# Medical-Image-Analysis-Laboratory/MSLesions3D

Measured on AMD Instinct MI355X. Metric: training volumes/sec at 128^3 batch-4 (fwd+loss+bwd+Adam), data-parallel over N MI355X, higher is better.
Workload: dtype f32; 1 GPU; 128^3 synthetic volumes, batch 4/GPU, 1 channel(s), fp32, SSD3D+MobileNet3D full train step (BASELINE configs[1]); global_batch=4, parallelism=dp1, priors=9344

## Files before the change

mslesions3d_amd/csrc/pwconv.hip:

```cpp
#include "common.hpp"
#include <algorithm>
#include <cstdlib>

namespace {

typedef float f32x16 __attribute__((ext_vector_type(16)));

constexpr int BM = 64, BN = 128, BK = 32;
constexpr int FOLD_MAXK = 512;
constexpr int WS_LD = BK + 1;

template <bool AFFINE, bool STATS, bool TRANS_W>
__global__ __launch_bounds__(256) void pw_gemm_kernel(const float* __restrict__ X,
                                                      const float* __restrict__ in_scale,
                                                      const float* __restrict__ in_shift,
                                                      const float* __restrict__ Wt, float* __restrict__ Y,
                                                      double* __restrict__ partials, int M, int K, int S,
                                                      msl::BnFold fold) {
  __shared__ __align__(16) float Xs[BK][BN];
  __shared__ float Ws[BM][WS_LD];
  __shared__ float red[2][2][BM];
  __shared__ float f_sc[AFFINE ? FOLD_MAXK : 1], f_sh[AFFINE ? FOLD_MAXK : 1];
  const int n = blockIdx.z, m0 = blockIdx.y * BM, s0 = blockIdx.x * BN;
  const int tid = threadIdx.x, lane = tid & 63, wv = tid >> 6;
  const int wm = wv >> 1, wn = wv & 1;
  const float* Xn = X + (size_t)n * K * S;
  const bool vec_ok = (S & 3) == 0;

  float4 xr[4], wr[2];
  auto load_chunk = [&](int k0) {
    if (vec_ok) {
#pragma unroll
      for (int i = 0; i < 4; ++i)
        xr[i] = msl::load4_zfill<true>(Xn + (size_t)(k0 + (tid >> 5) + i * 8) * S, s0 + (tid & 31) * 4, S);
    } else {
#pragma unroll
      for (int i = 0; i < 4; ++i)
        xr[i] = msl::load4_zfill<false>(Xn + (size_t)(k0 + (tid >> 5) + i * 8) * S, s0 + (tid & 31) * 4, S);
    }
#pragma unroll
    for (int i = 0; i < 2; ++i) {
      if (!TRANS_W) {
        const int m = (tid >> 3) + i * 32, k4 = (tid & 7) * 4;
        wr[i] = *reinterpret_cast<const float4*>(Wt + (size_t)(m0 + m < M ? m0 + m : 0) * K + k0 + k4);
      } else {
        const int k = (tid >> 4) + i * 16, m4 = (tid & 15) * 4;
        wr[i] = *reinterpret_cast<const float4*>(Wt + (size_t)(k0 + k) * M + (m0 + m4 < M ? m0 + m4 : 0));
      }
    }
  };
  auto store_chunk = [&](int k0) {
#pragma unroll
    for (int i = 0; i < 4; ++i) {
      const int r = (tid >> 5) + i * 8, c4 = (tid & 31) * 4, col = s0 + c4;
      float4 v = xr[i];
      if (AFFINE) {
        const float sc = f_sc[k0 + r], sh = f_sh[k0 + r];
        v.x = col < S ? msl::act(v.x, sc, sh) : 0.f;
        v.y = col + 1 < S ? msl::act(v.y, sc, sh) : 0.f;
        v.z = col + 2 < S ? msl::act(v.z, sc, sh) : 0.f;
        v.w = col + 3 < S ? msl::act(v.w, sc, sh) : 0.f;
      }
      *reinterpret_cast<float4*>(&Xs[r][c4]) = v;
    }
#pragma unroll
    for (int i = 0; i < 2; ++i) {
      const float4 v = wr[i];
      if (!TRANS_W) {
        const int m = (tid >> 3) + i * 32, k4 = (tid & 7) * 4;
        Ws[m][k4] = v.x; Ws[m][k4 + 1] = v.y; Ws[m][k4 + 2] = v.z; Ws[m][k4 + 3] = v.w;
      } else {
        const int k = (tid >> 4) + i * 16, m4 = (tid & 15) * 4;
        Ws[m4][k] = v.x; Ws[m4 + 1][k] = v.y; Ws[m4 + 2][k] = v.z; Ws[m4 + 3][k] = v.w;
      }
    }
  };

  f32x16 acc0 = {0}, acc1 = {0};
  load_chunk(0);
  if (AFFINE) {
    if (fold.partials) {
      msl::bn_fold_block(fold, 0, K, f_sc, f_sh);
    } else {
      for (int k = threadIdx.x; k < K && k < FOLD_MAXK; k += blockDim.x) {
        f_sc[k] = in_scale[k];
        f_sh[k] = in_shift[k];
      }
    }
  }
  for (int k0 = 0; k0 < K; k0 += BK) {
    __syncthreads();
    store_chunk(k0);
    __syncthreads();
    if (k0 + BK < K) load_chunk(k0 + BK);
#pragma unroll
    for (int kk = 0; kk < BK / 2; ++kk) {
      const int kr = 2 * kk + (lane >> 5);
      const float a = Ws[wm * 32 + (lane & 31)][kr];
      const float b0 = Xs[kr][wn * 64 + (lane & 31)];
      const float b1 = Xs[kr][wn * 64 + 32 + (lane & 31)];
      acc0 = __builtin_amdgcn_mfma_f32_32x32x2f32(a, b0, acc0, 0, 0, 0);
      acc1 = __builtin_amdgcn_mfma_f32_32x32x2f32(a, b1, acc1, 0, 0, 0);
    }
  }

  float* Yn = Y + (size_t)n * M * S;
  const int colbase = s0 + wn * 64 + (lane & 31);
#pragma unroll
  for (int r = 0; r < 16; ++r) {
    const int row = m0 + wm * 32 + (r & 3) + 8 * (r >> 2) + 4 * (lane >> 5);
    if (row < M && colbase < S) Yn[(size_t)row * S + colbase] = acc0[r];
    if (row < M && colbase + 32 < S) Yn[(size_t)row * S + colbase + 32] = acc1[r];
  }
  if (STATS) {
#pragma unroll
    for (int r = 0; r < 16; ++r) {
      float s = acc0[r] + acc1[r];
      float q = fmaf(acc0[r], acc0[r], acc1[r] * acc1[r]);
#pragma unroll
      for (int m = 16; m > 0; m >>= 1) {
        s += __shfl_xor(s, m, 64);
        q += __shfl_xor(q, m, 64);
      }
      if ((lane & 31) == 0) {
        const int row = wm * 32 + (r & 3) + 8 * (r >> 2) + 4 * (lane >> 5);
        red[0][wn][row] = s;
        red[1][wn][row] = q;
      }
    }
    __syncthreads();
    if (tid < BM && m0 + tid < M && partials) {
      const int NP = gridDim.z * gridDim.x, p = n * gridDim.x + blockIdx.x;
      partials[(size_t)(m0 + tid) * NP + p] = (double)red[0][0][tid] + (double)red[0][1][tid];
      partials[((size_t)M + m0 + tid) * NP + p] = (double)red[1][0][tid] + (double)red[1][1][tid];
    }
  }
}

constexpr int KS_BM = 32, KS_BN = 64;
constexpr int KS_WAVE_LDS = BK * KS_BN + KS_BM * WS_LD;

template <bool AFFINE, bool STATS, bool TRANS_W, int NW>
__global__ __launch_bounds__(NW * 64) void pw_gemm_ksplit_kernel(const float* __restrict__ X,
                                                             const float* __restrict__ in_scale,
                                                             const float* __restrict__ in_shift,
                                                             const float* __restrict__ Wt, float* __restrict__ Y,
                                                             double* __restrict__ partials, int M, int K, int S,
                                                             msl::BnFold fold) {
  extern __shared__ __align__(16) float lds[];
  __shared__ float f_sc[AFFINE ? FOLD_MAXK : 1], f_sh[AFFINE ? FOLD_MAXK : 1];
  const int n = blockIdx.z, m0 = blockIdx.y * KS_BM, s0 = blockIdx.x * KS_BN;
  const int tid = threadIdx.x, lane = tid & 63, wv = tid >> 6;
  float* Xs = lds + wv * KS_WAVE_LDS;
  float* Ws = Xs + BK * KS_BN;
  const float* Xn = X + (size_t)n * K * S;
  const bool vec_ok = (S & 3) == 0;
  const int kq = K / NW;
  const int kbeg = wv * kq;
  const int nchunks = kq / BK;

  float4 xr[8], wr[4];
  auto load_chunk = [&](int k0) {
    if (vec_ok) {
#pragma unroll
      for (int i = 0; i < 8; ++i)
        xr[i] = msl::load4_zfill<true>(Xn + (size_t)(k0 + (lane >> 4) + i * 4) * S, s0 + (lane & 15) * 4, S);
    } else {
#pragma unroll
      for (int i = 0; i < 8; ++i)
        xr[i] = msl::load4_zfill<false>(Xn + (size_t)(k0 + (lane >> 4) + i * 4) * S, s0 + (lane & 15) * 4, S);
    }
#pragma unroll
    for (int i = 0; i < 4; ++i) {
      if (!TRANS_W) {
        const int m = (lane >> 3) + i * 8, k4 = (lane & 7) * 4;
        wr[i] = *reinterpret_cast<const float4*>(Wt + (size_t)(m0 + m < M ? m0 + m : 0) * K + k0 + k4);
      } else {
        const int k = (lane >> 3) + i * 8, m4 = (lane & 7) * 4;
        wr[i] = *reinterpret_cast<const float4*>(Wt + (size_t)(k0 + k) * M + (m0 + m4 < M ? m0 + m4 : 0));
      }
    }
  };
  auto store_chunk = [&](int k0) {
#pragma unroll
    for (int i = 0; i < 8; ++i) {
      const int r = (lane >> 4) + i * 4, c4 = (lane & 15) * 4, col = s0 + c4;
      float4 v = xr[i];
      if (AFFINE) {
        const float sc = f_sc[k0 + r], sh = f_sh[k0 + r];
        v.x = col < S ? msl::act(v.x, sc, sh) : 0.f;
        v.y = col + 1 < S ? msl::act(v.y, sc, sh) : 0.f;
        v.z = col + 2 < S ? msl::act(v.z, sc, sh) : 0.f;
        v.w = col + 3 < S ? msl::act(v.w, sc, sh) : 0.f;
      }
      *reinterpret_cast<float4*>(Xs + r * KS_BN + c4) = v;
    }
#pragma unroll
    for (int i = 0; i < 4; ++i) {
      if (!TRANS_W) {
        const int m = (lane >> 3) + i * 8, k4 = (lane & 7) * 4;
        float* d = Ws + m * WS_LD + k4;
        d[0] = wr[i].x; d[1] = wr[i].y; d[2] = wr[i].z; d[3] = wr[i].w;
      } else {
        const int k = (lane >> 3) + i * 8, m4 = (lane & 7) * 4;
        Ws[(m4 + 0) * WS_LD + k] = wr[i].x; Ws[(m4 + 1) * WS_LD + k] = wr[i].y;
        Ws[(m4 + 2) * WS_LD + k] = wr[i].z; Ws[(m4 + 3) * WS_LD + k] = wr[i].w;
      }
    }
  };

  f32x16 acc0 = {0}, acc1 = {0};
  load_chunk(kbeg);
  if (AFFINE) {
    if (fold.partials) {
      msl::bn_fold_block(fold, 0, K, f_sc, f_sh);
    } else {
      for (int k = threadIdx.x; k < K && k < FOLD_MAXK; k += blockDim.x) {
        f_sc[k] = in_scale[k];
        f_sh[k] = in_shift[k];
      }
    }
  }
  for (int ch = 0; ch < nchunks; ++ch) {
    __syncthreads();
    store_chunk(kbeg + ch * BK);
    __syncthreads();
    if (ch + 1 < nchunks) load_chunk(kbeg + (ch + 1) * BK);
#pragma unroll
    for (int kk = 0; kk < BK / 2; ++kk) {
      const int kr = 2 * kk + (lane >> 5);
      const float a = Ws[(lane & 31) * WS_LD + kr];
      const float b0 = Xs[kr * KS_BN + (lane & 31)];
      const float b1 = Xs[kr * KS_BN + 32 + (lane & 31)];
      acc0 = __builtin_amdgcn_mfma_f32_32x32x2f32(a, b0, acc0, 0, 0, 0);
      acc1 = __builtin_amdgcn_mfma_f32_32x32x2f32(a, b1, acc1, 0, 0, 0);
    }
  }
  __syncthreads();
  constexpr int RLD = KS_BN + 1;
  for (int half = NW / 2; half >= 1; half >>= 1) {
    if (wv >= half && wv < 2 * half) {
      float* slot = lds + (wv - half) * (KS_BM * RLD);
#pragma unroll
      for (int r = 0; r < 16; ++r) {
        const int row = (r & 3) + 8 * (r >> 2) + 4 * (lane >> 5);
        slot[row * RLD + (lane & 31)] = acc0[r];
        slot[row * RLD + 32 + (lane & 31)] = acc1[r];
      }
    }
    __syncthreads();
    if (wv < half) {
      const float* slot = lds + wv * (KS_BM * RLD);
#pragma unroll
      for (int r = 0; r < 16; ++r) {
        const int row = (r & 3) + 8 * (r >> 2) + 4 * (lane >> 5);
        acc0[r] += slot[row * RLD + (lane & 31)];
        acc1[r] += slot[row * RLD + 32 + (lane & 31)];
      }
    }
    __syncthreads();
  }
  if (wv != 0) return;
  float* Yn = Y + (size_t)n * M * S;
  const int colbase = s0 + (lane & 31);
#pragma unroll
  for (int r = 0; r < 16; ++r) {
    const int rl = (r & 3) + 8 * (r >> 2) + 4 * (lane >> 5);
    const int row = m0 + rl;
    const float v0 = acc0[r];
    const float v1 = acc1[r];
    if (row < M && colbase < S) Yn[(size_t)row * S + colbase] = v0;
    if (row < M && colbase + 32 < S) Yn[(size_t)row * S + colbase + 32] = v1;
    if (STATS) {
      float s = v0 + v1;
      float q = fmaf(v0, v0, v1 * v1);
#pragma unroll
      for (int m = 16; m > 0; m >>= 1) {
        s += __shfl_xor(s, m, 64);
        q += __shfl_xor(q, m, 64);
      }
      if ((lane & 31) == 0 && row < M && partials) {
        const int NP = gridDim.z * gridDim.x, p = n * gridDim.x + blockIdx.x;
        partials[(size_t)row * NP + p] = (double)s;
        partials[((size_t)M + row) * NP + p] = (double)q;
      }
    }
  }
}

constexpr int WV_LD = 33;

template <int KW, int MT, bool AFFINE, bool STATS, bool TRANS_W, int NWK, int NT = 1>
__global__ __launch_bounds__(NWK == 1 ? 256 : NWK * 64) void pw_wave_kernel(
    const float* __restrict__ X, const float* __restrict__ in_scale, const float* __restrict__ in_shift,
    const float* __restrict__ Wt, float* __restrict__ Y, double* __restrict__ partials, int M, int K, int S,
    msl::BnFold fold) {
  constexpr int KH = KW / 2;
  static_assert(NWK == 1 || (MT == 1 && NT == 1), "the K-split form owns one tile");
  __shared__ float red[NWK == 1 ? 2 * 4 * MT * 32 : NWK * 32 * WV_LD];
  __shared__ float f_sc[AFFINE ? FOLD_MAXK : 1], f_sh[AFFINE ? FOLD_MAXK : 1];
  const int lane = threadIdx.x & 63, wv = threadIdx.x >> 6, h = lane >> 5, c = lane & 31;
  const int n = blockIdx.z;
  const int m0 = blockIdx.y * 32 * MT;
  const int ctile = NWK == 1 ? (blockIdx.x * 4 + wv) * NT : blockIdx.x;
  const int kb = (NWK == 1 ? 0 : wv * KW) + h * KH;
  int col[NT];
  bool cin[NT];
  float xr[NT][KH], wr[MT][KH];
#pragma unroll
  for (int nt = 0; nt < NT; ++nt) {
    col[nt] = (ctile + nt) * 32 + c;
    cin[nt] = col[nt] < S;
    const float* xp = X + ((size_t)n * K + kb) * S + (cin[nt] ? col[nt] : S - 1);
#pragma unroll
    for (int kk = 0; kk < KH; ++kk) xr[nt][kk] = xp[(size_t)kk * S];
  }
#pragma unroll
  for (int mt = 0; mt < MT; ++mt) {
    if (!TRANS_W) {
      const float4* wp = reinterpret_cast<const float4*>(Wt + (size_t)(m0 + mt * 32 + c) * K + kb);
#pragma unroll
      for (int j = 0; j < KH / 4; ++j) {
        const float4 t = wp[j];
        wr[mt][4 * j] = t.x; wr[mt][4 * j + 1] = t.y; wr[mt][4 * j + 2] = t.z; wr[mt][4 * j + 3] = t.w;
      }
    } else {
      const float* wp = Wt + (size_t)kb * M + m0 + mt * 32 + c;
#pragma unroll
      for (int kk = 0; kk < KH; ++kk) wr[mt][kk] = wp[(size_t)kk * M];
    }
  }
  __builtin_amdgcn_sched_barrier(0);
  if (AFFINE) {
    if (fold.partials) {
      msl::bn_fold_block(fold, 0, K, f_sc, f_sh);
#pragma unroll
      for (int nt = 0; nt < NT; ++nt)
#pragma unroll
        for (int kk = 0; kk < KH; ++kk) xr[nt][kk] = cin[nt] ? msl::act(xr[nt][kk], f_sc[kb + kk], f_sh[kb + kk]) : 0.f;
    } else {
      float sc[KH], sh[KH];
      const float4* sp = reinterpret_cast<const float4*>(in_scale + kb);
      const float4* hp = reinterpret_cast<const float4*>(in_shift + kb);
#pragma unroll
      for (int j = 0; j < KH / 4; ++j) {
        const float4 a = sp[j], b = hp[j];
        sc[4 * j] = a.x; sc[4 * j + 1] = a.y; sc[4 * j + 2] = a.z; sc[4 * j + 3] = a.w;
        sh[4 * j] = b.x; sh[4 * j + 1] = b.y; sh[4 * j + 2] = b.z; sh[4 * j + 3] = b.w;
      }
#pragma unroll
      for (int nt = 0; nt < NT; ++nt)
#pragma unroll
        for (int kk = 0; kk < KH; ++kk) xr[nt][kk] = cin[nt] ? msl::act(xr[nt][kk], sc[kk], sh[kk]) : 0.f;
    }
  } else {
#pragma unroll
    for (int nt = 0; nt < NT; ++nt)
#pragma unroll
      for (int kk = 0; kk < KH; ++kk) xr[nt][kk] = cin[nt] ? xr[nt][kk] : 0.f;
  }

  f32x16 acc[MT][NT];
#pragma unroll
  for (int mt = 0; mt < MT; ++mt)
#pragma unroll
    for (int nt = 0; nt < NT; ++nt) acc[mt][nt] = (f32x16){0};
#pragma unroll
  for (int kk = 0; kk < KH; ++kk)
#pragma unroll
    for (int mt = 0; mt < MT; ++mt)
#pragma unroll
      for (int nt = 0; nt < NT; ++nt)
        acc[mt][nt] = __builtin_amdgcn_mfma_f32_32x32x2f32(wr[mt][kk], xr[nt][kk], acc[mt][nt], 0, 0, 0);

  float* Yn = Y + (size_t)n * M * S;
  const int NP = gridDim.z * gridDim.x, p = n * gridDim.x + blockIdx.x;
  if (NWK == 1) {
#pragma unroll
    for (int mt = 0; mt < MT; ++mt)
#pragma unroll
      for (int r = 0; r < 16; ++r) {
        const int row = mt * 32 + (r & 3) + 8 * (r >> 2) + 4 * h;
        float v = 0.f, v2 = 0.f;
#pragma unroll
        for (int nt = 0; nt < NT; ++nt) {
          const float a = acc[mt][nt][r];
          if (cin[nt]) Yn[(size_t)(m0 + row) * S + col[nt]] = a;
          v += a;
          v2 = fmaf(a, a, v2);
        }
        if (STATS) {
          const float sm = msl::half32_sum(v), q = msl::half32_sum(v2);
          if (c == msl::HALF32_SUM_LANE) {
            red[(wv * MT * 32 + row) * 2] = sm;
            red[(wv * MT * 32 + row) * 2 + 1] = q;
          }
        }
      }
    if (STATS) {
      __syncthreads();
      const int t = threadIdx.x;
      if (t < MT * 32 && partials) {
        double sm = 0.0, q = 0.0;
#pragma unroll
        for (int w2 = 0; w2 < 4; ++w2) {
          sm += (double)red[(w2 * MT * 32 + t) * 2];
          q += (double)red[(w2 * MT * 32 + t) * 2 + 1];
        }
        partials[(size_t)(m0 + t) * NP + p] = sm;
        partials[((size_t)M + m0 + t) * NP + p] = q;
      }
    }
  } else {
    float* mine = red + wv * 32 * WV_LD;
#pragma unroll
    for (int r = 0; r < 16; ++r) mine[((r & 3) + 8 * (r >> 2) + 4 * h) * WV_LD + c] = acc[0][0][r];
    __syncthreads();
    constexpr int RPW = 32 / NWK;
#pragma unroll
    for (int e = 0; e < RPW / 2; ++e) {
      const int row = wv * RPW + 2 * e + h;
      float v = 0.f;
#pragma unroll
      for (int j = 0; j < NWK; ++j) v += red[(j * 32 + row) * WV_LD + c];
      if (cin[0]) Yn[(size_t)(m0 + row) * S + col[0]] = v;
      if (STATS) {
        const float sm = msl::half32_sum(v), q = msl::half32_sum(v * v);
        if (c == msl::HALF32_SUM_LANE && partials) {
          partials[(size_t)(m0 + row) * NP + p] = (double)sm;
          partials[((size_t)M + m0 + row) * NP + p] = (double)q;
        }
      }
    }
  }
}

template <int K, int COLS, int MT, bool AFFINE, bool STATS, bool TRANS_W>
__global__ __launch_bounds__(256) void pw_strip_kernel(const float* __restrict__ X, const float* __restrict__ in_scale,
                                                       const float* __restrict__ in_shift, const float* __restrict__ Wt,
                                                       float* __restrict__ Y, double* __restrict__ partials, int S,
                                                       msl::BnFold fold) {
  constexpr int M = 32 * MT, CT = COLS / 32, TPW = MT * CT / 4, KH = K / 2;
  static_assert(TPW >= 1 && (TPW <= CT) && CT % TPW == 0, "a wave owns TPW column tiles of one row tile");
  constexpr int LPT = K * COLS / 4 / 256;
  constexpr int C4 = COLS / 4;
  __shared__ __align__(16) float Xs[K * COLS];
  __shared__ float f_sc[AFFINE ? K : 1], f_sh[AFFINE ? K : 1];
  __shared__ float rs[(STATS && TPW != CT) ? 4 * 32 * 2 : 1];
  const int n = blockIdx.y, s0 = blockIdx.x * COLS;
  const int tid = threadIdx.x, lane = tid & 63, wv = tid >> 6, h = lane >> 5, c = lane & 31;
  const int t0 = wv * TPW, mt = t0 / CT, ct0 = t0 % CT;
  const int m0 = mt * 32;
  const float* Xn = X + (size_t)n * K * S + s0;
  typedef float f32x4v __attribute__((ext_vector_type(4)));
  f32x4v xv[LPT];
  const int r0 = tid / C4, c4 = (tid % C4) * 4;
#pragma unroll
  for (int i = 0; i < LPT; ++i) xv[i] = *reinterpret_cast<const f32x4v*>(Xn + (size_t)(r0 + i * (256 / C4)) * S + c4);
  float wr[KH];
  if (!TRANS_W) {
    const f32x4v* wp = reinterpret_cast<const f32x4v*>(Wt + (size_t)(m0 + c) * K + h * KH);
#pragma unroll
    for (int j = 0; j < KH / 4; ++j) {
      const f32x4v t = wp[j];
      wr[4 * j] = t.x; wr[4 * j + 1] = t.y; wr[4 * j + 2] = t.z; wr[4 * j + 3] = t.w;
    }
  } else {
    const float* wp = Wt + (size_t)(h * KH) * M + m0 + c;
#pragma unroll
    for (int kk = 0; kk < KH; ++kk) wr[kk] = wp[(size_t)kk * M];
  }
  __builtin_amdgcn_sched_barrier(0);
  if (AFFINE) {
    if (fold.partials) {
      msl::bn_fold_block(fold, 0, K, f_sc, f_sh);
    } else {
      if (tid < K) {
        f_sc[tid] = in_scale[tid];
        f_sh[tid] = in_shift[tid];
      }
      __syncthreads();
    }
  }
#pragma unroll
  for (int i = 0; i < LPT; ++i) {
    const int r = r0 + i * (256 / C4);
    f32x4v v = xv[i];
    if (AFFINE) {
      const float sc = f_sc[r], sh = f_sh[r];
      v.x = msl::act(v.x, sc, sh); v.y = msl::act(v.y, sc, sh); v.z = msl::act(v.z, sc, sh); v.w = msl::act(v.w, sc, sh);
    }
    *reinterpret_cast<f32x4v*>(&Xs[r * COLS + c4]) = v;
  }
  __syncthreads();
  f32x16 acc[TPW];
#pragma unroll
  for (int t = 0; t < TPW; ++t) acc[t] = (f32x16){0};
  const float* xb = Xs + (size_t)(h * KH) * COLS + ct0 * 32 + c;
#pragma unroll
  for (int kk = 0; kk < KH; ++kk)
#pragma unroll
    for (int t = 0; t < TPW; ++t) acc[t] = __builtin_amdgcn_mfma_f32_32x32x2f32(wr[kk], xb[kk * COLS + t * 32], acc[t], 0, 0, 0);
  float* Yn = Y + (size_t)n * M * S + s0 + ct0 * 32 + c;
  const int NP = gridDim.y * gridDim.x, p = n * gridDim.x + blockIdx.x;
#pragma unroll
  for (int r = 0; r < 16; ++r) {
    const int row = m0 + (r & 3) + 8 * (r >> 2) + 4 * h;
    float v = 0.f, v2 = 0.f;
#pragma unroll
    for (int t = 0; t < TPW; ++t) {
      const float a = acc[t][r];
      Yn[(size_t)row * S + t * 32] = a;
      v += a;
      v2 = fmaf(a, a, v2);
    }
    if (STATS) {
      const float sm = msl::half32_sum(v), q = msl::half32_sum(v2);
      if (TPW == CT) {
        if (c == msl::HALF32_SUM_LANE && partials) {
          partials[(size_t)row * NP + p] = (double)sm;
          partials[((size_t)M + row) * NP + p] = (double)q;
        }
      } else if (c == msl::HALF32_SUM_LANE) {
        rs[(wv * 32 + row - m0) * 2] = sm;
        rs[(wv * 32 + row - m0) * 2 + 1] = q;
      }
    }
  }
  if (STATS && TPW != CT) {
    constexpr int PW = CT / TPW;
    __syncthreads();
    if (tid < M && partials) {
      const int w0 = (tid / 32) * PW, rl = tid % 32;
      double sm = 0.0, q = 0.0;
#pragma unroll
      for (int u = 0; u < PW; ++u) {
        sm += (double)rs[((w0 + u) * 32 + rl) * 2];
        q += (double)rs[((w0 + u) * 32 + rl) * 2 + 1];
      }
      partials[(size_t)tid * NP + p] = sm;
      partials[((size_t)M + tid) * NP + p] = q;
    }
  }
}

static inline int strip_cols(int N, int K, int M, int S) {
  constexpr int on = 1;
  if (!on) return 0;
  int cols = 0;
  if (K == 32 && M == 64) cols = 256;
  else if (K == 64 && M == 32) cols = 128;
  else if ((K == 64 && M == 128) || (K == 128 && (M == 128 || M == 64))) cols = 64;
  if (!cols || S % cols != 0 || (long long)N * (S / cols) < 128) return 0;
  return cols;
}

template <bool AFFINE, bool STATS, bool TRANS_W>
static int launch_strip(const float* X, const float* in_scale, const float* in_shift, const float* Wt, float* Y,
                        double* partials, int N, int M, int K, int S, int cols, const msl::BnFold& fold, hipStream_t st) {
  dim3 grid(S / cols, N);
#define MSL_ST(K_, C_, MT_) \
  MSL_LAUNCH((pw_strip_kernel<K_, C_, MT_, AFFINE, STATS, TRANS_W>), grid, dim3(256), 0, st, X, in_scale, in_shift, Wt, Y, partials, S, fold)
  if (K == 32 && M == 64) MSL_ST(32, 256, 2);
  else if (K == 64 && M == 32) MSL_ST(64, 128, 1);
  else if (K == 64 && M == 128) MSL_ST(64, 64, 4);
  else if (K == 128 && M == 128) MSL_ST(128, 64, 4);
  else if (K == 128 && M == 64) MSL_ST(128, 64, 2);
  else return MSL_ERR_UNSUPPORTED;
#undef MSL_ST
  MSL_LAUNCH_CHECK();
  return MSL_OK;
}

static inline int wave_nt(int N, int K, int M, int S) {
  constexpr int force = 0;
  if (K > 64) return 1;
  if (force) return force;
  const int mt = (M % 64 == 0) ? 2 : 1;
  const long long waves = (long long)N * msl::cdiv(S, 32) * (M / (32 * mt));
  return waves >= 4096 ? 2 : 1;
}

static inline int wave_form(int K, int M) {
  if (M % 32 != 0) return 0;
  if (K == 32) return 32;
  if (K == 64 || K == 128 || K == 256 || K == 512) return 64;
  return 0;
}

template <bool AFFINE, bool STATS, bool TRANS_W>
static int launch_wave(const float* X, const float* in_scale, const float* in_shift, const float* Wt, float* Y,
                       double* partials, int N, int M, int K, int S, const msl::BnFold& fold, hipStream_t st) {
#define MSL_WV(KW_, MT_, NWK_)                                                                                        \
  MSL_LAUNCH((pw_wave_kernel<KW_, MT_, AFFINE, STATS, TRANS_W, NWK_>),                                        \
                     dim3(msl::cdiv(S, NWK_ == 1 ? 128 : 32), M / (32 * MT_), N), dim3(NWK_ == 1 ? 256 : NWK_ * 64), \
                     0, st, X, in_scale, in_shift, Wt, Y, partials, M, K, S, fold)
#define MSL_WV1(KW_, MT_)                                                                                              \
  do {                                                                                                                 \
    if (nt == 2)                                                                                                       \
      MSL_LAUNCH((pw_wave_kernel<KW_, MT_, AFFINE, STATS, TRANS_W, 1, 2>), dim3(msl::cdiv(S, 256), M / (32 * MT_), N), \
                         dim3(256), 0, st, X, in_scale, in_shift, Wt, Y, partials, M, K, S, fold);                     \
    else                                                                                                               \
      MSL_WV(KW_, MT_, 1);                                                                                             \
  } while (0)
  const bool two = M % 64 == 0;
  const int nt = STATS ? wave_nt(N, K, M, S) : 1;
  if (K == 32) {
    if (two) MSL_WV1(32, 2); else MSL_WV1(32, 1);
  } else if (K == 64) {
    if (two) MSL_WV1(64, 2); else MSL_WV1(64, 1);
  } else {
    switch (K / 64) {
      case 2: MSL_WV(64, 1, 2); break;
      case 4: MSL_WV(64, 1, 4); break;
      case 8: MSL_WV(64, 1, 8); break;
      default: return MSL_ERR_UNSUPPORTED;
    }
  }
#undef MSL_WV1
#undef MSL_WV
  MSL_LAUNCH_CHECK();
  return MSL_OK;
}

constexpr int PC = 64, PC_LD = PC + 1;

template <int BNN, bool AFFINE>
__global__ __launch_bounds__(256) void pw_bwd_weight_kernel(const float* __restrict__ dY,
                                                            const float* __restrict__ Z,
                                                            const float* __restrict__ in_scale,
                                                            const float* __restrict__ in_shift,
                                                            float* __restrict__ slabs, int Cout, int Cin,
                                                            int S, int N, int chunks_per_img,
                                                            int chunks_per_block) {
  constexpr int NSUB_N = BNN / 32;
  constexpr int NSUB = 2 * NSUB_N;
  __shared__ __align__(16) float lds[(64 + BNN) * PC_LD > 64 * BNN ? (64 + BNN) * PC_LD : 64 * BNN];
  float* dys = lds;
  float* as_ = lds + 64 * PC_LD;
  const int ks = blockIdx.x;
  const int tiles_n = Cin / BNN;
  const int tm = blockIdx.y / tiles_n, tn = blockIdx.y % tiles_n;
  const int m0 = tm * 64, n0 = tn * BNN;
  const int tid = threadIdx.x, lane = tid & 63, wv = tid >> 6;
  const int total_chunks = N * chunks_per_img;
  const int ch_lo = ks * chunks_per_block, ch_hi = min(total_chunks, ch_lo + chunks_per_block);
  const bool vec_ok = (S & 3) == 0;

  f32x16 acc[NSUB];
#pragma unroll
  for (int i = 0; i < NSUB; ++i) acc[i] = (f32x16){0};

  float scv[BNN / 16], shv[BNN / 16];
#pragma unroll
  for (int j = 0; j < BNN / 16; ++j) {
    scv[j] = AFFINE ? in_scale[n0 + (tid >> 4) + j * 16] : 1.f;
    shv[j] = AFFINE ? in_shift[n0 + (tid >> 4) + j * 16] : 0.f;
  }

  for (int ch = ch_lo; ch < ch_hi; ++ch) {
    const int n = ch / chunks_per_img, s0 = (ch % chunks_per_img) * PC;
    const float* dyn = dY + ((size_t)n * Cout + m0) * S;
    const float* zn = Z + ((size_t)n * Cin + n0) * S;
    float4 st[(64 + BNN) / 16];
    if (vec_ok) {
#pragma unroll
      for (int i = 0; i < (64 + BNN) / 16; ++i) {
        const int r = (tid >> 4) + i * 16;
        st[i] = msl::load4_zfill<true>(r < 64 ? dyn + (size_t)r * S : zn + (size_t)(r - 64) * S, s0 + (tid & 15) * 4, S);
      }
    } else {
#pragma unroll
      for (int i = 0; i < (64 + BNN) / 16; ++i) {
        const int r = (tid >> 4) + i * 16;
        st[i] = msl::load4_zfill<false>(r < 64 ? dyn + (size_t)r * S : zn + (size_t)(r - 64) * S, s0 + (tid & 15) * 4, S);
      }
    }
#pragma unroll
    for (int i = 0; i < (64 + BNN) / 16; ++i) {
      const int r = (tid >> 4) + i * 16, c4 = (tid & 15) * 4, col = s0 + c4;
      float4 v = st[i];
      if (AFFINE && r >= 64) {
        const float sc = scv[i >= 4 ? i - 4 : 0], sh = shv[i >= 4 ? i - 4 : 0];
        v.x = col < S ? msl::act(v.x, sc, sh) : 0.f;
        v.y = col + 1 < S ? msl::act(v.y, sc, sh) : 0.f;
        v.z = col + 2 < S ? msl::act(v.z, sc, sh) : 0.f;
        v.w = col + 3 < S ? msl::act(v.w, sc, sh) : 0.f;
      }
      float* dst = lds + r * PC_LD + c4;
      dst[0] = v.x; dst[1] = v.y; dst[2] = v.z; dst[3] = v.w;
    }
    __syncthreads();
#pragma unroll
    for (int kk = 0; kk < 8; ++kk) {
      const int pos = wv * 16 + 2 * kk + (lane >> 5);
      float a[2], b[NSUB_N];
#pragma unroll
      for (int i = 0; i < 2; ++i) a[i] = dys[(i * 32 + (lane & 31)) * PC_LD + pos];
#pragma unroll
      for (int j = 0; j < NSUB_N; ++j) b[j] = as_[(j * 32 + (lane & 31)) * PC_LD + pos];
#pragma unroll
      for (int i = 0; i < 2; ++i)
#pragma unroll
        for (int j = 0; j < NSUB_N; ++j)
          acc[i * NSUB_N + j] = __builtin_amdgcn_mfma_f32_32x32x2f32(a[i], b[j], acc[i * NSUB_N + j], 0, 0, 0);
    }
    __syncthreads();
  }

  float* redt = lds;
  for (int w = 3; w >= 1; --w) {
    if (wv == w) {
#pragma unroll
      for (int i = 0; i < 2; ++i)
#pragma unroll
        for (int j = 0; j < NSUB_N; ++j)
#pragma unroll
          for (int r = 0; r < 16; ++r) {
            const int row = i * 32 + (r & 3) + 8 * (r >> 2) + 4 * (lane >> 5);
            const int col = j * 32 + (lane & 31);
            const float v = acc[i * NSUB_N + j][r];
            if (w == 3) redt[row * BNN + col] = v;
            else redt[row * BNN + col] += v;
          }
    }
    __syncthreads();
  }
  if (wv == 0) {
    float* out = slabs + (size_t)ks * Cout * Cin;
#pragma unroll
    for (int i = 0; i < 2; ++i)
#pragma unroll
      for (int j = 0; j < NSUB_N; ++j)
#pragma unroll
        for (int r = 0; r < 16; ++r) {
          const int row = i * 32 + (r & 3) + 8 * (r >> 2) + 4 * (lane >> 5);
          const int col = j * 32 + (lane & 31);
          out[(size_t)(m0 + row) * Cin + n0 + col] = acc[i * NSUB_N + j][r] + redt[row * BNN + col];
        }
  }
}

template <int MT, bool AFFINE>
__device__ __forceinline__ void pw_bww_wave_body(const float* __restrict__ dY, const float* __restrict__ Z,
                                                 const float* __restrict__ in_scale, const float* __restrict__ in_shift,
                                                 float* __restrict__ out, int Cout, int Cin, int S, int chunks_per_img,
                                                 int total_chunks, int chunks_per_block, int ks, int tile) {
  __shared__ __align__(16) float red[4 * MT * 1024];
  const int lane = threadIdx.x & 63, wv = threadIdx.x >> 6, h = lane >> 5, c = lane & 31;
  const int tiles_n = Cin / 32;
  const int tm = tile / tiles_n, tn = tile % tiles_n;
  const int m0 = tm * 32 * MT, n0 = tn * 32;
  const int ch_lo = ks * chunks_per_block, ch_hi = min(total_chunks, ch_lo + chunks_per_block);
  const int mine = max(0, (ch_hi - ch_lo - wv + 3) / 4);

  float sc = 1.f, sh = 0.f;
  if (AFFINE) {
    sc = in_scale[n0 + c];
    sh = in_shift[n0 + c];
  }
  f32x16 acc[MT];
#pragma unroll
  for (int mt = 0; mt < MT; ++mt) acc[mt] = (f32x16){0};

  float4 a0[MT][4], b0[4], a1[MT][4], b1[4];
  auto issue = [&](int i, float4 (&a)[MT][4], float4 (&b)[4]) {
    const int ch = min(ch_lo + wv + 4 * i, total_chunks - 1);
    const int n = ch / chunks_per_img, s0 = (ch - n * chunks_per_img) * 32 + 16 * h;
#pragma unroll
    for (int mt = 0; mt < MT; ++mt) {
      const float4* p = reinterpret_cast<const float4*>(dY + ((size_t)n * Cout + m0 + mt * 32 + c) * S + s0);
#pragma unroll
      for (int j = 0; j < 4; ++j) a[mt][j] = p[j];
    }
    const float4* q = reinterpret_cast<const float4*>(Z + ((size_t)n * Cin + n0 + c) * S + s0);
#pragma unroll
    for (int j = 0; j < 4; ++j) b[j] = q[j];
  };
  auto mac = [&](float4 (&a)[MT][4], float4 (&b)[4]) {
#pragma unroll
    for (int j = 0; j < 4; ++j) {
      float bv[4] = {b[j].x, b[j].y, b[j].z, b[j].w};
#pragma unroll
      for (int e = 0; e < 4; ++e) {
        const float x = AFFINE ? msl::act(bv[e], sc, sh) : bv[e];
#pragma unroll
        for (int mt = 0; mt < MT; ++mt) {
          const float av = e == 0 ? a[mt][j].x : e == 1 ? a[mt][j].y : e == 2 ? a[mt][j].z : a[mt][j].w;
          acc[mt] = __builtin_amdgcn_mfma_f32_32x32x2f32(av, x, acc[mt], 0, 0, 0);
        }
      }
    }
  };

  if (mine > 0) issue(0, a0, b0);
#pragma unroll 1
  for (int i = 0; i < mine; i += 2) {
    issue(i + 1, a1, b1);
    __builtin_amdgcn_sched_barrier(0);
    mac(a0, b0);
    if (i + 1 < mine) {
      issue(i + 2, a0, b0);
      __builtin_amdgcn_sched_barrier(0);
      mac(a1, b1);
    }
  }

#pragma unroll
  for (int mt = 0; mt < MT; ++mt)
#pragma unroll
    for (int r = 0; r < 16; ++r) red[((wv * MT + mt) * 32 + (r & 3) + 8 * (r >> 2) + 4 * h) * 32 + c] = acc[mt][r];
  __syncthreads();
  float* dst = out + (size_t)ks * Cout * Cin;
#pragma unroll
  for (int e = 0; e < MT; ++e) {
    const int q4 = threadIdx.x + e * 256;
    const int row = q4 >> 3, col = (q4 & 7) * 4;
    float4 v = *reinterpret_cast<const float4*>(&red[(0 * MT * 32 + row) * 32 + col]);
#pragma unroll
    for (int w2 = 1; w2 < 4; ++w2) {
      const float4 t = *reinterpret_cast<const float4*>(&red[(w2 * MT * 32 + row) * 32 + col]);
      v.x += t.x; v.y += t.y; v.z += t.z; v.w += t.w;
    }
    *reinterpret_cast<float4*>(dst + (size_t)(m0 + row) * Cin + n0 + col) = v;
  }
}

template <int MT, bool AFFINE>
__global__ __launch_bounds__(256) void pw_bww_wave_kernel(const float* __restrict__ dY, const float* __restrict__ Z,
                                                          const float* __restrict__ in_scale,
                                                          const float* __restrict__ in_shift, float* __restrict__ out,
                                                          int Cout, int Cin, int S, int chunks_per_img, int total_chunks,
                                                          int chunks_per_block) {
  pw_bww_wave_body<MT, AFFINE>(dY, Z, in_scale, in_shift, out, Cout, Cin, S, chunks_per_img, total_chunks, chunks_per_block,
                               blockIdx.x, blockIdx.y);
}

constexpr int PW_BWW_BATCH_MAX = 4;
struct PwBwwBatch {
  const float* dY[PW_BWW_BATCH_MAX];
  const float* Z[PW_BWW_BATCH_MAX];
  const float* in_scale[PW_BWW_BATCH_MAX];
  const float* in_shift[PW_BWW_BATCH_MAX];
  float* out[PW_BWW_BATCH_MAX];
  int Cout[PW_BWW_BATCH_MAX], Cin[PW_BWW_BATCH_MAX], S[PW_BWW_BATCH_MAX], chunks_per_img[PW_BWW_BATCH_MAX],
      total_chunks[PW_BWW_BATCH_MAX], chunks_per_block[PW_BWW_BATCH_MAX], ksplit[PW_BWW_BATCH_MAX],
      first[PW_BWW_BATCH_MAX + 1];
};

__global__ __launch_bounds__(256) void pw_bww_wave_batch_kernel(PwBwwBatch b, int n) {
  int k = 0;
#pragma unroll
  for (int j = 1; j < PW_BWW_BATCH_MAX; ++j)
    if (j < n && (int)blockIdx.x >= b.first[j]) k = j;
  const int local = blockIdx.x - b.first[k];
  pw_bww_wave_body<2, true>(b.dY[k], b.Z[k], b.in_scale[k], b.in_shift[k], b.out[k], b.Cout[k], b.Cin[k], b.S[k],
                            b.chunks_per_img[k], b.total_chunks[k], b.chunks_per_block[k], local % b.ksplit[k],
                            local / b.ksplit[k]);
}

struct BwwWavePlan {
  int mt, tiles, chunks_per_img, total_chunks, ksplit, chunks_per_block;
};

static inline bool bww_wave_plan(int N, int Cin, int Cout, int S, BwwWavePlan& p) {
  constexpr int off = 1;
  if (!off || S % 32 != 0 || Cin % 32 != 0 || Cout % 32 != 0) return false;
  p.mt = (Cout % 64 == 0) ? 2 : 1;
  p.tiles = (Cout / (32 * p.mt)) * (Cin / 32);
  p.chunks_per_img = S / 32;
  p.total_chunks = N * p.chunks_per_img;
  constexpr int target = 256;
  int ks = std::max(1, std::min(target / std::max(1, p.tiles), p.total_chunks / 8));
  p.chunks_per_block = msl::cdiv(p.total_chunks, ks);
  p.ksplit = msl::cdiv(p.total_chunks, p.chunks_per_block);
  return true;
}

__global__ __launch_bounds__(256) void slab_reduce_kernel(const float* __restrict__ slabs, float* __restrict__ out,
                                                          int count, int nslabs) {
  __shared__ float lds[8 * 33];
  const float t = msl::reduce_slabs_256(slabs, (size_t)count, count, nslabs, lds);
  const int i = blockIdx.x * 32 + (threadIdx.x & 31);
  if ((threadIdx.x >> 5) == 0 && i < count) out[i] = t;
}

struct BwPlan {
  int bnn, ksplit, chunks_per_img, chunks_per_block;
};

BwPlan bw_plan(int N, int Cin, int Cout, int S) {
  BwPlan p;
  p.bnn = (Cin % 64 == 0) ? 64 : 32;
  p.chunks_per_img = msl::cdiv(S, PC);
  const int total = N * p.chunks_per_img;
  const int tiles = (Cout / 64) * (Cin / p.bnn);
  int ks = std::max(1, std::min(total, 512 / std::max(1, tiles)));
  constexpr int min_cpb = 1;
  ks = std::max(1, std::min(ks, total / std::max(1, min_cpb)));
  p.chunks_per_block = msl::cdiv(total, ks);
  p.ksplit = msl::cdiv(total, p.chunks_per_block);
  return p;
}

}

extern "C" {

static inline bool use_ksplit(int K, int M, int S, int N) {
  return K >= 128 && K % 128 == 0 && msl::cdiv(S, BN) * msl::cdiv(M, BM) * N < 256;
}

int msl_pwconv_fwd_num_partials(int N, int Cin, int Cout, int S) {
  if (const int cols = strip_cols(N, Cin, Cout, S)) return N * (S / cols);
  if (wave_form(Cin, Cout)) return N * msl::cdiv(S, Cin <= 64 ? 128 * wave_nt(N, Cin, Cout, S) : 32);
  return N * msl::cdiv(S, use_ksplit(Cin, Cout, S, N) ? KS_BN : BN);
}

static const msl::BnFold pw_nofold{nullptr, 0, 0, 1.0, nullptr, nullptr, 0.f};

static int pwconv_fwd_impl(const float* z, const float* in_scale, const float* in_shift, const msl::BnFold& fold,
                           const float* w, float* y, double* partials, int N, int Cin, int Cout, int S, void* stream) {
  if (N <= 0 || S <= 0 || Cin % BK != 0 || Cout % 4 != 0) return MSL_ERR_ARG;
  if ((in_scale || fold.partials) && Cin > FOLD_MAXK) return MSL_ERR_UNSUPPORTED;
  hipStream_t st = (hipStream_t)stream;
  if (const int cols = strip_cols(N, Cin, Cout, S)) {
    if (in_scale || fold.partials) {
      if (partials) return launch_strip<true, true, false>(z, in_scale, in_shift, w, y, partials, N, Cout, Cin, S, cols, fold, st);
      return launch_strip<true, false, false>(z, in_scale, in_shift, w, y, partials, N, Cout, Cin, S, cols, fold, st);
    }
    if (partials) return launch_strip<false, true, false>(z, in_scale, in_shift, w, y, partials, N, Cout, Cin, S, cols, fold, st);
    return launch_strip<false, false, false>(z, in_scale, in_shift, w, y, partials, N, Cout, Cin, S, cols, fold, st);
  }
  if (wave_form(Cin, Cout)) {
    if (in_scale || fold.partials) {
      if (partials) return launch_wave<true, true, false>(z, in_scale, in_shift, w, y, partials, N, Cout, Cin, S, fold, st);
      return launch_wave<true, false, false>(z, in_scale, in_shift, w, y, partials, N, Cout, Cin, S, fold, st);
    }
    if (partials) return launch_wave<false, true, false>(z, in_scale, in_shift, w, y, partials, N, Cout, Cin, S, fold, st);
    return launch_wave<false, false, false>(z, in_scale, in_shift, w, y, partials, N, Cout, Cin, S, fold, st);
  }
  if (use_ksplit(Cin, Cout, S, N)) {
    dim3 g2(msl::cdiv(S, KS_BN), msl::cdiv(Cout, KS_BM), N);
#define MSL_KS(A_, S_, T_, X_, Wp_, Y_, P_, M_, K_)                                                                  \
  do {                                                                                                             \
    if ((K_) % 256 == 0) {                                                                                         \
      const size_t lds_ = (size_t)8 * KS_WAVE_LDS * sizeof(float);                                                 \
      hipError_t e_ = hipFuncSetAttribute(reinterpret_cast<const void*>(pw_gemm_ksplit_kernel<A_, S_, T_, 8>),    \
                                          hipFuncAttributeMaxDynamicSharedMemorySize, (int)lds_);                  \
      if (e_ != hipSuccess) return (int)e_;                                                                        \
      MSL_LAUNCH((pw_gemm_ksplit_kernel<A_, S_, T_, 8>), g2, dim3(512), lds_, st, X_, in_scale, in_shift,  \
                         Wp_, Y_, P_, M_, K_, S, fold);                                                            \
    } else {                                                                                                       \
      MSL_LAUNCH((pw_gemm_ksplit_kernel<A_, S_, T_, 4>), g2, dim3(256),                                    \
                         (size_t)4 * KS_WAVE_LDS * sizeof(float), st, X_, in_scale, in_shift, Wp_, Y_, P_, M_, K_, S, fold); \
    }                                                                                                              \
  } while (0)
    if (in_scale || fold.partials) {
      if (partials) MSL_KS(true, true, false, z, w, y, partials, Cout, Cin);
      else MSL_KS(true, false, false, z, w, y, partials, Cout, Cin);
    } else {
      if (partials) MSL_KS(false, true, false, z, w, y, partials, Cout, Cin);
      else MSL_KS(false, false, false, z, w, y, partials, Cout, Cin);
    }
    MSL_LAUNCH_CHECK();
    return MSL_OK;
  }
  dim3 grid(msl::cdiv(S, BN), msl::cdiv(Cout, BM), N);
  if (in_scale || fold.partials) {
    if (partials) MSL_LAUNCH((pw_gemm_kernel<true, true, false>), grid, dim3(256), 0, st, z, in_scale, in_shift, w, y, partials, Cout, Cin, S, fold);
    else MSL_LAUNCH((pw_gemm_kernel<true, false, false>), grid, dim3(256), 0, st, z, in_scale, in_shift, w, y, partials, Cout, Cin, S, fold);
  } else {
    if (partials) MSL_LAUNCH((pw_gemm_kernel<false, true, false>), grid, dim3(256), 0, st, z, in_scale, in_shift, w, y, partials, Cout, Cin, S, fold);
    else MSL_LAUNCH((pw_gemm_kernel<false, false, false>), grid, dim3(256), 0, st, z, in_scale, in_shift, w, y, partials, Cout, Cin, S, fold);
  }
  MSL_LAUNCH_CHECK();
  return MSL_OK;
}

int msl_pwconv_fwd(const float* z, const float* in_scale, const float* in_shift, const float* w, float* y,
                   double* partials, int N, int Cin, int Cout, int S, void* stream) {
  return pwconv_fwd_impl(z, in_scale, in_shift, pw_nofold, w, y, partials, N, Cin, Cout, S, stream);
}

int msl_pwconv_fwd_fold(const float* z, const double* in_partials, int in_np, double in_count, const float* gamma,
                        const float* beta, float eps, const float* w, float* y, double* partials, int N, int Cin,
                        int Cout, int S, void* stream) {
  if (!in_partials || in_np <= 0) return MSL_ERR_ARG;
  const msl::BnFold fold{in_partials, in_np, Cin, in_count, gamma, beta, eps};
  return pwconv_fwd_impl(z, nullptr, nullptr, fold, w, y, partials, N, Cin, Cout, S, stream);
}

int msl_pwconv_bwd_data(const float* dy, const float* w, float* g_in, int N, int Cin, int Cout, int S,
                        void* stream) {
  if (N <= 0 || S <= 0 || Cout % BK != 0 || Cin % 4 != 0) return MSL_ERR_ARG;
  if (const int cols = strip_cols(N, Cout, Cin, S))
    return launch_strip<false, false, true>(dy, nullptr, nullptr, w, g_in, nullptr, N, Cin, Cout, S, cols, pw_nofold,
                                            (hipStream_t)stream);
  if (wave_form(Cout, Cin))
    return launch_wave<false, false, true>(dy, nullptr, nullptr, w, g_in, nullptr, N, Cin, Cout, S, pw_nofold,
                                           (hipStream_t)stream);
  if (use_ksplit(Cout, Cin, S, N)) {
    dim3 g2(msl::cdiv(S, KS_BN), msl::cdiv(Cin, KS_BM), N);
    hipStream_t st = (hipStream_t)stream;
    const float *in_scale = nullptr, *in_shift = nullptr;
    double* nopart = nullptr;
    const msl::BnFold fold = pw_nofold;
    MSL_KS(false, false, true, dy, w, g_in, nopart, Cin, Cout);
    MSL_LAUNCH_CHECK();
    return MSL_OK;
  }
  dim3 grid(msl::cdiv(S, BN), msl::cdiv(Cin, BM), N);
  MSL_LAUNCH((pw_gemm_kernel<false, false, true>), grid, dim3(256), 0, (hipStream_t)stream, dy, nullptr,
                     nullptr, w, g_in, nullptr, Cin, Cout, S, pw_nofold);
  MSL_LAUNCH_CHECK();
  return MSL_OK;
}

size_t msl_pwconv_bwd_weight_workspace_bytes(int N, int Cin, int Cout, int S) {
  BwwWavePlan wp;
  if (bww_wave_plan(N, Cin, Cout, S, wp)) return (size_t)wp.ksplit * Cout * Cin * sizeof(float);
  BwPlan p = bw_plan(N, Cin, Cout, S);
  return (size_t)p.ksplit * Cout * Cin * sizeof(float);
}

int msl_pwconv_bwd_weight_nslabs(int N, int Cin, int Cout, int S) {
  BwwWavePlan wp;
  if (bww_wave_plan(N, Cin, Cout, S, wp)) return wp.ksplit;
  return bw_plan(N, Cin, Cout, S).ksplit;
}

int msl_pwconv_bwd_weight_slabs(const float* dy, const float* z, const float* in_scale, const float* in_shift,
                                float* out, int N, int Cin, int Cout, int S, void* stream) {
  if (N <= 0 || S <= 0 || Cin % 32 != 0 || Cout % 32 != 0) return MSL_ERR_ARG;
  hipStream_t st = (hipStream_t)stream;
  BwwWavePlan wp;
  if (bww_wave_plan(N, Cin, Cout, S, wp)) {
    dim3 grid(wp.ksplit, wp.tiles);
#define MSL_BWW(MT_, A_)                                                                                          \
  MSL_LAUNCH((pw_bww_wave_kernel<MT_, A_>), grid, dim3(256), 0, st, dy, z, in_scale, in_shift, out, Cout, Cin, \
                     S, wp.chunks_per_img, wp.total_chunks, wp.chunks_per_block)
    if (wp.mt == 2) {
      if (in_scale) MSL_BWW(2, true); else MSL_BWW(2, false);
    } else {
      if (in_scale) MSL_BWW(1, true); else MSL_BWW(1, false);
    }
#undef MSL_BWW
    MSL_LAUNCH_CHECK();
    return MSL_OK;
  }
  if (Cout % 64 != 0) return MSL_ERR_ARG;
  BwPlan p = bw_plan(N, Cin, Cout, S);
  dim3 grid(p.ksplit, (Cout / 64) * (Cin / p.bnn));
  if (p.bnn == 64) {
    if (in_scale) MSL_LAUNCH((pw_bwd_weight_kernel<64, true>), grid, dim3(256), 0, st, dy, z, in_scale, in_shift, out, Cout, Cin, S, N, p.chunks_per_img, p.chunks_per_block);
    else MSL_LAUNCH((pw_bwd_weight_kernel<64, false>), grid, dim3(256), 0, st, dy, z, in_scale, in_shift, out, Cout, Cin, S, N, p.chunks_per_img, p.chunks_per_block);
  } else {
    if (in_scale) MSL_LAUNCH((pw_bwd_weight_kernel<32, true>), grid, dim3(256), 0, st, dy, z, in_scale, in_shift, out, Cout, Cin, S, N, p.chunks_per_img, p.chunks_per_block);
    else MSL_LAUNCH((pw_bwd_weight_kernel<32, false>), grid, dim3(256), 0, st, dy, z, in_scale, in_shift, out, Cout, Cin, S, N, p.chunks_per_img, p.chunks_per_block);
  }
  MSL_LAUNCH_CHECK();
  return MSL_OK;
}

int msl_pwconv_bwd_weight_batchable(int N, int Cin, int Cout, int S) {
  BwwWavePlan wp;
  return (N > 0 && S > 0 && bww_wave_plan(N, Cin, Cout, S, wp) && wp.mt == 2) ? 1 : 0;
}

int msl_pwconv_bwd_weight_slabs_batch(const float* const* dy, const float* const* z, const float* const* in_scale,
                                      const float* const* in_shift, float* const* out, const int* Cin, const int* Cout,
                                      const int* S, int n, int N, void* stream) {
  if (n < 1 || n > PW_BWW_BATCH_MAX || N <= 0) return MSL_ERR_ARG;
  PwBwwBatch b;
  int total = 0;
  for (int k = 0; k < n; ++k) {
    BwwWavePlan wp;
    if (!dy[k] || !z[k] || !in_scale[k] || !in_shift[k] || !out[k]) return MSL_ERR_ARG;
    if (S[k] <= 0 || !bww_wave_plan(N, Cin[k], Cout[k], S[k], wp) || wp.mt != 2) return MSL_ERR_UNSUPPORTED;
    b.dY[k] = dy[k]; b.Z[k] = z[k]; b.in_scale[k] = in_scale[k]; b.in_shift[k] = in_shift[k]; b.out[k] = out[k];
    b.Cout[k] = Cout[k]; b.Cin[k] = Cin[k]; b.S[k] = S[k];
    b.chunks_per_img[k] = wp.chunks_per_img; b.total_chunks[k] = wp.total_chunks;
    b.chunks_per_block[k] = wp.chunks_per_block; b.ksplit[k] = wp.ksplit;
    b.first[k] = total;
    total += wp.ksplit * wp.tiles;
  }
  for (int k = n; k <= PW_BWW_BATCH_MAX; ++k) b.first[k] = total;
  for (int k = n; k < PW_BWW_BATCH_MAX; ++k) {
    b.dY[k] = b.Z[k] = b.in_scale[k] = b.in_shift[k] = nullptr; b.out[k] = nullptr;
    b.Cout[k] = b.Cin[k] = b.S[k] = b.chunks_per_img[k] = b.total_chunks[k] = b.chunks_per_block[k] = 0; b.ksplit[k] = 1;
  }
  MSL_LAUNCH(pw_bww_wave_batch_kernel, dim3(total), dim3(256), 0, (hipStream_t)stream, b, n);
  MSL_LAUNCH_CHECK();
  return MSL_OK;
}

int msl_pwconv_bwd_weight(const float* dy, const float* z, const float* in_scale, const float* in_shift,
                          float* dw, float* workspace, int N, int Cin, int Cout, int S, void* stream) {
  const int nslabs = msl_pwconv_bwd_weight_nslabs(N, Cin, Cout, S);
  if (nslabs == 1) return msl_pwconv_bwd_weight_slabs(dy, z, in_scale, in_shift, dw, N, Cin, Cout, S, stream);
  const int rc = msl_pwconv_bwd_weight_slabs(dy, z, in_scale, in_shift, workspace, N, Cin, Cout, S, stream);
  if (rc != MSL_OK) return rc;
  const int count = Cout * Cin;
  MSL_LAUNCH(slab_reduce_kernel, dim3(msl::cdiv(count, 32)), dim3(256), 0, (hipStream_t)stream, workspace, dw,
                     count, nslabs);
  MSL_LAUNCH_CHECK();
  return MSL_OK;
}

}
```

Baseline: 6152 volumes/s.

## Add double-buffered pipelined strip kernel for K=32,M=64 pointwise conv

Adds a new strip kernel variant that prefetches every column tile of X into registers up front, then stages the tiles one by one into a double-buffered LDS region while the MFMA loop for the previous tile runs. Only the K=32, M=64 case is routed to it. The aim is to hide global load latency behind the matrix math and shrink the LDS footprint. In exchange it holds more registers for the prefetched tiles, which may lower occupancy.

```diff
diff --git a/mslesions3d_amd/csrc/pwconv.hip b/mslesions3d_amd/csrc/pwconv.hip
--- a/mslesions3d_amd/csrc/pwconv.hip
+++ b/mslesions3d_amd/csrc/pwconv.hip
@@ -544,6 +544,135 @@
   }
 }
 
+template <int K, int COLS, int MT, bool AFFINE, bool STATS, bool TRANS_W>
+__global__ __launch_bounds__(256) void pw_strip_pipe_kernel(const float* __restrict__ X, const float* __restrict__ in_scale,
+                                                            const float* __restrict__ in_shift,
+                                                            const float* __restrict__ Wt, float* __restrict__ Y,
+                                                            double* __restrict__ partials, int S, msl::BnFold fold) {
+  constexpr int M = 32 * MT, CT = COLS / 32, TPW = MT * CT / 4, KH = K / 2;
+  static_assert(TPW > 1 && TPW <= CT && CT % TPW == 0, "a wave owns TPW > 1 column tiles of one row tile");
+  constexpr int PW = CT / TPW;
+  constexpr int SC = 32 * PW;
+  constexpr int Q = SC / 4;
+  constexpr int RPP = 256 / Q;
+  constexpr int LPS = K / RPP;
+  static_assert(256 % Q == 0 && K % RPP == 0 && LPS >= 1, "whole rows per pass");
+  __shared__ __align__(16) float Xs[2][K * SC];
+  __shared__ float f_sc[AFFINE ? K : 1], f_sh[AFFINE ? K : 1];
+  __shared__ float rs[(STATS && PW != 1) ? 4 * 32 * 2 : 1];
+  const int n = blockIdx.y, s0 = blockIdx.x * COLS;
+  const int tid = threadIdx.x, lane = tid & 63, wv = tid >> 6, h = lane >> 5, c = lane & 31;
+  const int t0 = wv * TPW, mt = t0 / CT, ct0 = t0 % CT, g = ct0 / TPW;
+  const int m0 = mt * 32;
+  typedef float f32x4v __attribute__((ext_vector_type(4)));
+  const int r0 = tid / Q, q = tid % Q;
+  const float* Xn = X + (size_t)n * K * S + s0 + (q / 8) * (TPW * 32) + (q % 8) * 4;
+  float wr[KH];
+  if (!TRANS_W) {
+    const f32x4v* wp = reinterpret_cast<const f32x4v*>(Wt + (size_t)(m0 + c) * K + h * KH);
+#pragma unroll
+    for (int j = 0; j < KH / 4; ++j) {
+      const f32x4v t = wp[j];
+      wr[4 * j] = t.x; wr[4 * j + 1] = t.y; wr[4 * j + 2] = t.z; wr[4 * j + 3] = t.w;
+    }
+  } else {
+    const float* wp = Wt + (size_t)(h * KH) * M + m0 + c;
+#pragma unroll
+    for (int kk = 0; kk < KH; ++kk) wr[kk] = wp[(size_t)kk * M];
+  }
+  float in_sc = 0.f, in_sh = 0.f;
+  if (AFFINE && !fold.partials && tid < K) {
+    in_sc = in_scale[tid];
+    in_sh = in_shift[tid];
+  }
+  __builtin_amdgcn_sched_barrier(0);
+  f32x4v xv[TPW][LPS];
+#pragma unroll
+  for (int j = 0; j < TPW; ++j)
+#pragma unroll
+    for (int i = 0; i < LPS; ++i) xv[j][i] = *reinterpret_cast<const f32x4v*>(Xn + (size_t)(r0 + i * RPP) * S + j * 32);
+  __builtin_amdgcn_sched_barrier(0);
+  if (AFFINE) {
+    if (fold.partials) {
+      msl::bn_fold_block(fold, 0, K, f_sc, f_sh);
+    } else {
+      if (tid < K) {
+        f_sc[tid] = in_sc;
+        f_sh[tid] = in_sh;
+      }
+      __syncthreads();
+    }
+  }
+  auto stage = [&](const f32x4v (&x)[LPS], float* dst) {
+#pragma unroll
+    for (int i = 0; i < LPS; ++i) {
+      const int r = r0 + i * RPP;
+      f32x4v v = x[i];
+      if (AFFINE) {
+        const float sc = f_sc[r], sh = f_sh[r];
+        v.x = msl::act(v.x, sc, sh); v.y = msl::act(v.y, sc, sh); v.z = msl::act(v.z, sc, sh); v.w = msl::act(v.w, sc, sh);
+      }
+      *reinterpret_cast<f32x4v*>(&dst[r * SC + q * 4]) = v;
+    }
+  };
+  stage(xv[0], Xs[0]);
+  __syncthreads();
+  float* Yn = Y + (size_t)n * M * S + s0 + ct0 * 32 + c;
+  float v[16], v2[16];
+#pragma unroll
+  for (int r = 0; r < 16; ++r) v[r] = v2[r] = 0.f;
+#pragma unroll
+  for (int j = 0; j < TPW; ++j) {
+    const float* xb = Xs[j & 1] + (h * KH) * SC + g * 32 + c;
+    f32x16 acc = (f32x16){0};
+#pragma unroll
+    for (int kk = 0; kk < KH; ++kk) acc = __builtin_amdgcn_mfma_f32_32x32x2f32(wr[kk], xb[kk * SC], acc, 0, 0, 0);
+#pragma unroll
+    for (int r = 0; r < 16; ++r) {
+      const int row = m0 + (r & 3) + 8 * (r >> 2) + 4 * h;
+      const float a = acc[r];
+      Yn[(size_t)row * S + j * 32] = a;
+      v[r] += a;
+      v2[r] = fmaf(a, a, v2[r]);
+    }
+    if (j + 1 < TPW) {
+      stage(xv[j + 1], Xs[(j + 1) & 1]);
+      __syncthreads();
+    }
+  }
+  if (STATS) {
+    const int NP = gridDim.y * gridDim.x, p = n * gridDim.x + blockIdx.x;
+#pragma unroll
+    for (int r = 0; r < 16; ++r) {
+      const int row = m0 + (r & 3) + 8 * (r >> 2) + 4 * h;
+      const float sm = msl::half32_sum(v[r]), sq = msl::half32_sum(v2[r]);
+      if (PW == 1) {
+        if (c == msl::HALF32_SUM_LANE && partials) {
+          partials[(size_t)row * NP + p] = (double)sm;
+          partials[((size_t)M + row) * NP + p] = (double)sq;
+        }
+      } else if (c == msl::HALF32_SUM_LANE) {
+        rs[(wv * 32 + row - m0) * 2] = sm;
+        rs[(wv * 32 + row - m0) * 2 + 1] = sq;
+      }
+    }
+    if (PW != 1) {
+      __syncthreads();
+      if (tid < M && partials) {
+        const int w0 = (tid / 32) * PW, rl = tid % 32;
+        double sm = 0.0, sq = 0.0;
+#pragma unroll
+        for (int u = 0; u < PW; ++u) {
+          sm += (double)rs[((w0 + u) * 32 + rl) * 2];
+          sq += (double)rs[((w0 + u) * 32 + rl) * 2 + 1];
+        }
+        partials[(size_t)tid * NP + p] = sm;
+        partials[((size_t)M + tid) * NP + p] = sq;
+      }
+    }
+  }
+}
+
 static inline int strip_cols(int N, int K, int M, int S) {
   constexpr int on = 1;
   if (!on) return 0;
@@ -561,12 +690,15 @@
   dim3 grid(S / cols, N);
 #define MSL_ST(K_, C_, MT_) \
   MSL_LAUNCH((pw_strip_kernel<K_, C_, MT_, AFFINE, STATS, TRANS_W>), grid, dim3(256), 0, st, X, in_scale, in_shift, Wt, Y, partials, S, fold)
-  if (K == 32 && M == 64) MSL_ST(32, 256, 2);
+#define MSL_STP(K_, C_, MT_) \
+  MSL_LAUNCH((pw_strip_pipe_kernel<K_, C_, MT_, AFFINE, STATS, TRANS_W>), grid, dim3(256), 0, st, X, in_scale, in_shift, Wt, Y, partials, S, fold)
+  if (K == 32 && M == 64) MSL_STP(32, 256, 2);
   else if (K == 64 && M == 32) MSL_ST(64, 128, 1);
   else if (K == 64 && M == 128) MSL_ST(64, 64, 4);
   else if (K == 128 && M == 128) MSL_ST(128, 64, 4);
   else if (K == 128 && M == 64) MSL_ST(128, 64, 2);
   else return MSL_ERR_UNSUPPORTED;
+#undef MSL_STP
 #undef MSL_ST
   MSL_LAUNCH_CHECK();
   return MSL_OK;
```

Result: no change. 6164 volumes/s, median of 4 (+0.2%).
